# pps-lab/rofl-project-code

Hardware: AMD Instinct MI355X
Metric: range-proof elements/sec (create+verify), d=25k 32-bit (higher is better)
Workload: dtype u32x8 (255-bit integer field)

## Files before the change

### rofl_project_code_amd/csrc/host_msm.hpp

```cpp
#pragma once

MsmPlan msm_plan(size_t n, size_t np = 1) {
    MsmPlan p;
    static const size_t t13 = knob("ROFL_MSM_T13") ? (size_t)atol(knob("ROFL_MSM_T13")) : ((size_t)1 << 13);
    static const size_t t10_knob = knob("ROFL_MSM_T10") ? (size_t)atol(knob("ROFL_MSM_T10")) : 0;
    const size_t t10 = t10_knob ? t10_knob : (np >= 32 ? (size_t)1 << 11 : (size_t)1 << 9);
    if (n >= (1u << 17)) p.c = 16; else if (n >= t13) p.c = 13; else if (n >= t10) p.c = 10; else if (n >= 64) p.c = 7; else p.c = 4;
    if (const char *e = knob("ROFL_MSM_C")) { int v = atoi(e); if (v == 4 || v == 7 || v == 10 || v == 13 || v == 16) p.c = (u32)v; }
    p.W = (254 + p.c - 1) / p.c;
    p.W = (253 - p.c + p.c - 1) / p.c + 1;
    p.wide = (253 - p.c) - (p.c - 1) * (p.W - 1);
    p.B = 1u << (p.c - 1);
    p.levels = (p.c - 1) / 3;
    return p;
}
struct MsmOpt { u32 lr_nh = 0, lr_ng = 0; const niels *fb_wtab = nullptr; size_t fb_stride = 0; u32 fb_c = 16; std::function<void()> overlap; std::function<void(size_t)> post; u32 tag = 0;
                std::function<void(size_t, int)> post8;
                const sc *ip_dev = nullptr; u32 ip_nblk = 0; const niels *qpts = nullptr; bool *ip_included = nullptr;
                hipEvent_t pts_ready = nullptr; };

struct MsmAllow { bool fb = true, small = true, two = true, slots = true; };
enum class MsmKind { FixedBase, Small, Slots, CountSort };
struct MsmJob {
    MsmWs *ws = nullptr; size_t np = 0, nq = 0, n = 0, PW = 0; MsmPlan P{}; MsmKind kind = MsmKind::CountSort; bool lr = false, two = false, dev_horner = false;
// ... 8 lines not shown
    static const int sigmas = knob("ROFL_MSM_BIN_SIGMA") ? atoi(knob("ROFL_MSM_BIN_SIGMA")) : 8;
    size_t hot = 2 * avg, dev = 1;
    if (sigmas <= 0) return (u32)((hot + 256 + 63) / 64 * 64);
    while (dev * dev < hot) dev++;
    return (u32)((hot + (size_t)sigmas * dev + 64 + 63) / 64 * 64);
}

bool msm_plan_job(Ctx &C, MsmJob &J, const MsmOpt &opt, const MsmAllow &al, MsmMap &mm, u32 &small_cap, Msm2L &tl) {
    const size_t np = J.np, n = J.n; const bool lr = J.lr; const size_t nq = J.nq;
    const size_t per_side = lr ? n / 2 : n;
    mm = MsmMap{opt.lr_nh, opt.lr_ng, 0, 0, 0};
    J.two = false; J.sets = 0;
    bool want_fb = al.fb && opt.fb_wtab != nullptr && C.msm_slots;
    if (want_fb) {
        J.kind = MsmKind::FixedBase;
        J.P = msm_plan_c(opt.fb_c);
        bool crowded = C.crowded();
        size_t want = crowded ? C.msm_fb_threads / 2 : C.msm_fb_threads;
        u32 sets = J.P.W;
        for (u32 sdiv = 1; sdiv <= J.P.W; sdiv++)
            if (J.P.W % sdiv == 0 && (size_t)nq * (lr ? 2 : 1) * sdiv * J.P.B >= want) { sets = sdiv; break; }
        static const bool fitsets = !(knob("ROFL_MSM_FB_FITSETS") && atoi(knob("ROFL_MSM_FB_FITSETS")) == 0);
        if (fitsets && al.two && C.msm_two_level && (J.P.B == 32768 || J.P.B == 16384) && per_side >= 8192)
            while (sets < J.P.W && (size_t)msm_bin_cap(per_side * (J.P.W / sets) / 512) * 4 + 1024 > 96 * 1024) {
                u32 nx = sets + 1; while (nx < J.P.W && J.P.W % nx) nx++;
                sets = nx;
            }
        J.sets = sets;
        mm.fb_sets = sets; mm.fb_wps = J.P.W / sets; mm.fb_stride = (u32)opt.fb_stride;
        J.PW = nq * (lr ? 2 : 1) * sets;
        u32 cap = 16; while (cap < 2048 && (size_t)cap * J.P.B < 3 * per_side * (mm.fb_wps + 1)) cap *= 2;
        if (mm.fb_wps == 1) cap *= 2;
        J.cap = cap;
        bool two = al.two && C.msm_two_level && J.P.W * opt.fb_stride <= ((size_t)1 << 24) && (J.P.B == 32768 || J.P.B == 16384);
        const u32 fb0 = J.P.B == 32768 ? 7u : 6u;
        tl = Msm2L{256, fb0, 24, 0, 144};
        if (two) {
            auto size_bins = [&]() { tl.cap_bin = msm_bin_cap(per_side * mm.fb_wps / tl.nbins); return (size_t)tl.cap_bin * 4 + 1024 <= 96 * 1024; };
            bool fits = size_bins();
            if (!fits) { tl = Msm2L{512, fb0 - 1, 24, 0, 72}; fits = size_bins(); }
            if (!fits || per_side < 8192) two = false;
        }
        J.two = two;
        if (!two && (size_t)J.PW * J.P.B * J.cap * 4 > ((size_t)8 << 30)) return false;
        return true;
    }
    bool slots_mode = al.slots && C.msm_slots;
    J.P = msm_plan(n, J.np);
    if (C.msm_small_max && al.small && slots_mode && per_side <= C.msm_small_max && J.P.c > 10 && np * 26 <= 512) J.P = msm_plan_c(10);
    J.PW = np * J.P.W;
    { u32 cap = 16; while (cap < 256 && (size_t)cap * J.P.B < 4 * n) cap *= 2; J.cap = cap; }
    small_cap = per_side <= 8 * J.P.B ? (u32)MSM_SMALL_CAP : 72u;
    size_t small_lds = std::max((size_t)J.P.B * 4 * (1 + small_cap), std::max(((size_t)(J.P.B / 8) * 4 + (size_t)(J.P.B / 16) * 5 + 1) * sizeof(ge), ((size_t)J.P.B + (size_t)J.P.B * 3 / 4 + 1) * sizeof(ge)));
    bool small = slots_mode && al.small && C.msm_small_max && per_side <= C.msm_small_max && J.P.c <= 10 && per_side <= 16 * J.P.B && (J.PW <= 512 || small_lds <= 24 * 1024);
    J.kind = small ? MsmKind::Small : slots_mode ? MsmKind::Slots : MsmKind::CountSort;
    J.small_group = 1;
    if (small && J.P.B == 64 && J.PW > 512) {
        static const u32 grp = knob("ROFL_MSM_SMALL_GROUP") ? (u32)std::max(1, std::min(4, atoi(knob("ROFL_MSM_SMALL_GROUP")))) : 4u;
        J.small_group = grp == 3 ? 2 : grp;
    }
    if (J.kind == MsmKind::Slots && (size_t)J.PW * J.P.B * J.cap * 4 > ((size_t)8 << 30)) return false;
    return true;
}

MsmJob msm_enqueue(Ctx &C, MsmWs &W, const std::vector<MsmProb> &probs, size_t n, const MsmOpt &opt, MsmAllow &al, hipStream_t st = nullptr) {
    if (!st) st = C.stream;
    static const u32 acc_balance = knob("ROFL_ACC_BALANCE") ? (atoi(knob("ROFL_ACC_BALANCE")) ? 1u : 0u) : 1u;
    static const u32 dbg_mask = knob("ROFL_DBG_IDX_MASK") ? (u32)strtoul(knob("ROFL_DBG_IDX_MASK"), nullptr, 0) : 0x7fffffffu;
    static const u32 dbg_scatter = knob("ROFL_DBG_SCATTER") ? (u32)atoi(knob("ROFL_DBG_SCATTER")) : 0u;
    MsmJob J; J.ws = &W; J.np = probs.size(); J.n = n; J.lr = opt.lr_nh != 0; J.nq = J.lr ? J.np / 2 : J.np;
    const size_t np = J.np, nq = J.nq; const bool lr = J.lr;
    MsmMap mm{}; u32 small_cap = 0; Msm2L tl{};
    while (!msm_plan_job(C, J, opt, al, mm, small_cap, tl)) {
        if (al.fb && opt.fb_wtab && C.msm_slots) al.fb = false; else al.slots = false;
    }
    const MsmPlan &P = J.P; const size_t PW = J.PW; const bool fb = J.fb();
    MsmProb *d_probs = W.probs.as<MsmProb>(np);
    MsmProb *h_probs = W.h_probs.as<MsmProb>(np);
    for (size_t i = 0; i < np; i++) h_probs[i] = fb ? MsmProb{opt.fb_wtab, probs[i].scal} : probs[i];
    if (W.probs_on_dev.size() != np || memcmp(W.probs_on_dev.data(), h_probs, sizeof(MsmProb) * np) != 0) {
        HIPCHK(hipMemcpyAsync(d_probs, h_probs, sizeof(MsmProb) * np, hipMemcpyHostToDevice, st));
        W.probs_on_dev.assign(h_probs, h_probs + np);
    }
    u32 *cnt = W.cnt.as<u32>(PW * P.B + 4), *off = W.off.as<u32>(PW * P.B), *cur = W.cur.as<u32>(PW * P.B);
    u32 *perm = W.perm.as<u32>(PW * P.B);
    ge *buckets = W.buckets.as<ge>(PW * P.B);
    MsmWin mw{P.c, P.W, P.wide};
    static const bool host8_on = h8::available() && !(knob("ROFL_MSM_HOST8") && atoi(knob("ROFL_MSM_HOST8")) == 0);
    static const size_t host8_min = knob("ROFL_MSM_HOST8_MIN") ? (size_t)std::max(1L, atol(knob("ROFL_MSM_HOST8_MIN"))) : 8;
    J.dev_horner = !fb && P.W <= 64 && (np >= C.msm_dev_horner_min || (host8_on && np >= host8_min));
    J.host8 = J.dev_horner && host8_on;
    ge *hres_dev = W.h_res.dev<ge>(PW * (size_t)P.c + np);
    u32 *h_flag = W.h_ovf.as<u32>(4), *d_flag = W.h_ovf.dev<u32>(4);
    const u32 Wb = (u32)(PW / nq);
    const u32 n_side = (u32)(lr ? n / 2 : n);
    const u32 nb_final = P.c - 1;
    hipEvent_t e0 = nullptr, e1 = nullptr;
    *h_flag = 0;
    if (opt.ip_included) *opt.ip_included = J.kind == MsmKind::Small && opt.ip_dev && opt.qpts && lr;
    if (J.kind == MsmKind::Small) {
        ge *S_fin_s = J.dev_horner ? W.S[0].as<ge>(PW) : hres_dev;
        ge *C_fin_s = J.dev_horner ? W.Cacc[0].as<ge>(PW * (size_t)nb_final) : hres_dev + PW;
        const u32 G = J.small_group;
        size_t lds_lists = G > 1 ? (size_t)G * P.B * (4 + 2 * (size_t)small_cap)
                                 : (size_t)P.B * 4 * (1 + small_cap);
        size_t lds_red = G > 1 ? ((size_t)G * P.B * 3 / 4 + 1) * sizeof(ge)
                               : std::max(((size_t)(P.B / 8) * 4 + (size_t)(P.B / 16) * 5 + 1) * sizeof(ge), ((size_t)P.B + (size_t)P.B * 3 / 4 + 1) * sizeof(ge));
        uint64_t items = (uint64_t)np * n_side * P.W;
        KSpan ks(C.tm, st, ROFL_TK_MSM_SMALL, items * 7 + (uint64_t)PW * P.B * 10, (uint64_t)np * n_side * (32 + 96));
        static const bool small_tl = knob("ROFL_DBG_SMALL_TIMELINE") != nullptr;
        unsigned long long *tl_dev = nullptr;
        if (small_tl) { HIPCHK(hipMalloc(&tl_dev, PW * 32)); HIPCHK(hipMemsetAsync(tl_dev, 0, PW * 32, st)); }
        if (opt.pts_ready) HIPCHK(hipStreamWaitEvent(st, opt.pts_ready, 0));
        const u32 Wg = (P.W + G - 1) / G;
        if (G > 1)
            ROFL_LAUNCH(k_msm_small_g, dim3((unsigned)(np * Wg)), dim3(G * P.B), std::max(lds_lists, lds_red), st, n_side, mw, mm, d_probs, buckets,
                               S_fin_s, C_fin_s, nb_final, d_flag, small_cap, G, tl_dev, J.host8 ? hres_dev : (ge *)nullptr,
                               lr ? opt.ip_dev : (const sc *)nullptr, opt.ip_nblk, lr ? opt.qpts : (const niels *)nullptr);
        else
            ROFL_LAUNCH(k_msm_small, dim3((unsigned)PW), dim3(P.B < 64 ? 64 : P.B), std::max(lds_lists, lds_red), st, n_side, mw, mm, d_probs, buckets,
                               S_fin_s, C_fin_s, nb_final, d_flag, small_cap, G, tl_dev, J.host8 ? hres_dev : (ge *)nullptr,
                               lr ? opt.ip_dev : (const sc *)nullptr, opt.ip_nblk, lr ? opt.qpts : (const niels *)nullptr);
        if (small_tl) {
            std::vector<unsigned long long> hts(PW * 4);
            HIPCHK(hipMemcpyAsync(hts.data(), tl_dev, PW * 32, hipMemcpyDeviceToHost, st)); HIPCHK(hipStreamSynchronize(st)); HIPCHK(hipFree(tl_dev));
            double ph[3] = {0, 0, 0}; unsigned long long t_lo = ~0ull, t_hi = 0;
            const size_t nblocks = G > 1 ? np * Wg : PW;
            for (size_t b = 0; b < nblocks; b++) { for (int k = 0; k < 3; k++) ph[k] += (double)(hts[b * 4 + k + 1] - hts[b * 4 + k]); t_lo = std::min(t_lo, hts[b * 4]); t_hi = std::max(t_hi, hts[b * 4 + 3]); }
            fprintf(stderr, "[rofl] k_msm_small PW=%zu blocks=%zu n_side=%u c=%u: rank %.1f us, bucket sums %.1f us, reduce %.1f us (block means); first start -> last end %.1f us\n",
                    PW, nblocks, n_side, P.c, ph[0] / nblocks * 0.01, ph[1] / nblocks * 0.01, ph[2] / nblocks * 0.01, (double)(t_hi - t_lo) * 0.01);
        }
        if (J.host8) {}
        else if (J.dev_horner) ROFL_LAUNCH(k_msm_horner, dim3((unsigned)np), dim3(256), 0, st, mw, (const ge *)S_fin_s, (const ge *)C_fin_s, nb_final, hres_dev);
        return J;
    }
    const uint64_t terms = (uint64_t)(lr ? nq : np) * n;
    if (J.two) {
        u32 *bins = W.sorted.as<u32>(PW * tl.nbins * tl.cap_bin);
        u32 *bcur = W.cur.as<u32>(PW * tl.nbins * 2);
        u32 *btail = W.tail.as<u32>(PW * tl.nbins * (size_t)MSM_BIN_TAIL);
        HIPCHK(hipMemsetAsync(bcur, 0, sizeof(u32) * PW * tl.nbins * 2, st));
        static const bool worder_on = !(knob("ROFL_MSM_WINDOW_ORDER") && atoi(knob("ROFL_MSM_WINDOW_ORDER")) == 0);
        const u64 wdiv = (u64)mm.fb_stride * mm.fb_sets;
        const bool worder = worder_on && mm.fb_wps > 1 && mm.fb_wps <= 16 && wdiv && (wdiv & (wdiv - 1)) == 0 && wdiv < ((u64)1 << tl.ebits);
        const u32 worder_wps = worder ? mm.fb_wps : 1u, worder_shift = worder ? (u32)lg2u((size_t)wdiv) : 0u;
        u32 iter_pts = (tl.stage >= 144 ? 16384u : 12288u) / mm.fb_wps; if (iter_pts < 1024) iter_pts = 1024;
        u32 tile = iter_pts;
        while (((size_t)((n_side + tile - 1) / tile) * PW > 512 || (n_side + tile - 1) / tile > 48) && tile < n_side) tile *= 2;
        {
            static const bool tile_search = !(knob("ROFL_MSM_BIN_TILE_SEARCH") && atoi(knob("ROFL_MSM_BIN_TILE_SEARCH")) == 0);
            const size_t kCU = 256;
            auto cost = [&](u32 t) { const size_t tiles = (n_side + t - 1) / t; return (double)((tiles * PW + kCU - 1) / kCU) * ((double)std::min<u32>(t, n_side) + 0.25 * iter_pts); };
            if (tile_search) {
                u32 best = tile; double best_cost = cost(tile);
                for (u32 t = iter_pts; t < n_side + iter_pts; t += iter_pts) {
                    const size_t tiles = (n_side + t - 1) / t;
                    if (tiles > 48 || tiles * PW > 4096) continue;
                    const double c = cost(t);
                    if (c < best_cost * 0.999) { best = t; best_cost = c; }
                }
                if (knob("ROFL_TRACE")) fprintf(stderr, "[rofl] bin_l1 tiling: n_side=%u PW=%zu iter=%u: tile %u (%zu blocks, cost %.0f) -> best %u (%zu blocks, cost %.0f)\n", n_side, PW, iter_pts, tile,
                                                (size_t)((n_side + tile - 1) / tile) * PW, cost(tile), best, (size_t)((n_side + best - 1) / best) * PW, best_cost);
                if (best_cost < 0.85 * cost(tile)) tile = best;
            }
        }
        dim3 grid((n_side + tile - 1) / tile, (u32)PW);
        { KSpan ks(C.tm, st, ROFL_TK_MSM_SCATTER, 0, terms * 32 + terms * P.W * 4);
          ROFL_LAUNCH(k_msm_bin_l1, grid, dim3(1024), (size_t)(tl.nbins + tl.nbins * tl.stage) * 4, st, n_side, tile, iter_pts, mw, mm, d_probs, bcur, bins, btail, tl, d_flag);
          ROFL_LAUNCH(k_msm_bin_l2, dim3(tl.nbins, (u32)PW), dim3(512), (size_t)(2 * 128 * worder_wps + tl.cap_bin) * 4, st, tl, P.B, bcur, bins, (const u32 *)btail, cnt, off, d_flag,
                      worder_wps, worder_shift); }
        ROFL_LAUNCH(k_msm_scan, dim3((unsigned)PW), dim3(P.B >= 1024 ? 1024 : 256), 0, st, P.B, cnt, off, (u32 *)nullptr, perm);
        if (C.tm.enabled) { e0 = C.tm.get(); e1 = C.tm.get(); HIPCHK(hipEventRecord(e0, st)); }
        {
            HeavyScope heavy(C, st); hipStream_t hst = heavy.run;
            KSpan ks_acc(C.tm, hst, ROFL_TK_MSM_ACCUMULATE_FB, terms * P.W * 7, terms * 32);
            static const char *timeline = knob("ROFL_DBG_ACC_TIMELINE");
            if (timeline) {
                dim3 g = grid1((size_t)Wb * P.B, (u32)nq);
                size_t waves = (size_t)g.x * g.y * (TPB / 64);
                unsigned long long *rec; HIPCHK(hipMalloc(&rec, waves * 32)); HIPCHK(hipMemsetAsync(rec, 0, waves * 32, st));
                ROFL_LAUNCH(k_msm_accumulate_fb_dbg, g, dim3(TPB), 0, st, (u32)n, P.c, Wb, (u32)(np / nq), d_probs, cnt, off, bins, perm, buckets, MSM_LIST_ABS, dbg_mask, acc_balance, rec);
                std::vector<unsigned long long> h(waves * 4);
                HIPCHK(hipMemcpyAsync(h.data(), rec, waves * 32, hipMemcpyDeviceToHost, st)); HIPCHK(hipStreamSynchronize(st));
                if (FILE *f = fopen(timeline, "ab")) { unsigned long long hdr[4] = {0x54494d45ull, waves, g.x, g.y}; fwrite(hdr, 8, 4, f); fwrite(h.data(), 8, h.size(), f); fclose(f); }
                HIPCHK(hipFree(rec));
            } else
            ROFL_LAUNCH(k_msm_accumulate_fb, grid1((size_t)Wb * P.B, (u32)nq), dim3(TPB), 0, hst, (u32)n, P.c, Wb, (u32)(np / nq), d_probs, cnt, off, bins, perm, buckets, MSM_LIST_ABS, dbg_mask,
                        acc_balance | ((worder && nq > 1 && Wb > 1) ? 2u : 0u));
        }
        if (C.tm.enabled) HIPCHK(hipEventRecord(e1, st));
    } else if (J.kind != MsmKind::CountSort) {
        HIPCHK(hipMemsetAsync(cnt, 0, sizeof(u32) * (PW * P.B + 4), st));
        const u32 cap = J.cap;
        u32 *slots = W.sorted.as<u32>(PW * P.B * cap);
        MsmOvf *ovf = W.ovf.as<MsmOvf>(MSM_OVF_MAX);
        u32 *ovf_count = cnt + PW * P.B;
        if (C.msm_lds && n >= C.msm_lds_min && (size_t)P.B * 4 <= 128 * 1024) {
            u32 per_q = fb ? J.sets : P.W;
            u32 tile = n_side;
            u32 wps = fb ? mm.fb_wps : 1;
            while (tile > 1024 && ((size_t)tile * wps > (size_t)C.msm_lds_tile || (size_t)((n_side + tile - 1) / tile) * nq * (lr ? 2 : 1) * per_q < 256)) tile /= 2;
            dim3 grid((n_side + tile - 1) / tile, (u32)(nq * (lr ? 2 : 1) * per_q));
            uint64_t items = terms * P.W;
            KSpan ks(C.tm, st, ROFL_TK_MSM_SCATTER, 0, terms * 32 + items * 4);
            ROFL_LAUNCH(k_msm_scatter_lds, grid, dim3(1024), (size_t)P.B * 4, st, n_side, tile, mw, mm, d_probs, cnt, slots, cap, ovf_count, ovf, MSM_OVF_MAX, dbg_scatter);
        } else
            ROFL_LAUNCH(k_msm_scatter_slots, grid1(n, (u32)(nq * P.W)), dim3(TPB), 0, st, (u32)n, mw, mm, d_probs, cnt, slots, cap, ovf_count, ovf, MSM_OVF_MAX);
        ROFL_LAUNCH(k_msm_scan, dim3((unsigned)PW), dim3(P.B >= 1024 ? 1024 : 256), 0, st, P.B, cnt, off, (u32 *)nullptr, perm);
        if (opt.pts_ready) HIPCHK(hipStreamWaitEvent(st, opt.pts_ready, 0));
        if (C.tm.enabled) { e0 = C.tm.get(); e1 = C.tm.get(); HIPCHK(hipEventRecord(e0, st)); }
        {
            uint64_t acc_adds = terms * P.W;
            const bool big = acc_adds >= ((uint64_t)1 << 22);
            HeavyScope heavy(C, st, big); hipStream_t hst = heavy.run;
            KSpan ks_acc(C.tm, hst, fb ? ROFL_TK_MSM_ACCUMULATE_FB : ROFL_TK_MSM_ACCUMULATE_GEN, acc_adds * 7, terms * 32);
            if (fb) ROFL_LAUNCH(k_msm_accumulate_fb, grid1((size_t)Wb * P.B, (u32)nq), dim3(TPB), 0, hst, (u32)n, P.c, Wb, (u32)(np / nq), d_probs, cnt, off, slots, perm, buckets, cap, dbg_mask, acc_balance);
            else ROFL_LAUNCH(k_msm_accumulate_gen, grid1((size_t)Wb * P.B, (u32)nq), dim3(TPB), 0, hst, (u32)n, P.c, Wb, (u32)(np / nq), d_probs, cnt, off, slots, perm, buckets, cap, dbg_mask, acc_balance);
        }
        if (C.tm.enabled) HIPCHK(hipEventRecord(e1, st));
        ROFL_LAUNCH(k_msm_overflow, dim3(1), dim3(64), 0, st, Wb, P.B, (u32)(np / nq), d_probs, ovf_count, ovf, MSM_OVF_MAX, buckets, fb ? 1 : 0);
        HIPCHK(hipMemcpyAsync(h_flag, ovf_count, 4, hipMemcpyDeviceToHost, st));
    } else {
        HIPCHK(hipMemsetAsync(cnt, 0, sizeof(u32) * (PW * P.B + 4), st));
        u32 *sorted = W.sorted.as<u32>(PW * n * 2);
        ROFL_LAUNCH(k_msm_count, grid1(n, (u32)(nq * P.W)), dim3(TPB), 0, st, (u32)n, mw, mm, d_probs, cnt);
        ROFL_LAUNCH(k_msm_scan, dim3((unsigned)PW), dim3(P.B >= 1024 ? 1024 : 256), 0, st, P.B, cnt, off, cur, perm);
        ROFL_LAUNCH(k_msm_scatter, grid1(n, (u32)(nq * P.W)), dim3(TPB), 0, st, (u32)n, mw, mm, d_probs, cur, sorted);
        if (opt.pts_ready) HIPCHK(hipStreamWaitEvent(st, opt.pts_ready, 0));
        if (C.tm.enabled) { e0 = C.tm.get(); e1 = C.tm.get(); HIPCHK(hipEventRecord(e0, st)); }
        ROFL_LAUNCH(k_msm_accumulate_gen, grid1((size_t)Wb * P.B, (u32)nq), dim3(TPB), 0, st, (u32)n, P.c, Wb, (u32)(np / nq), d_probs, cnt, off, sorted, perm, buckets, 0u, dbg_mask, acc_balance);
        if (C.tm.enabled) HIPCHK(hipEventRecord(e1, st));
    }
    if (C.tm.enabled) {
        C.tm.acc_ev.push_back({e0, e1}); C.tm.t.msm_accumulate_launches++; C.tm.t.msm_additions += terms * P.W;
        char tg[96]; snprintf(tg, sizeof tg, "msm np=%zu n=%zu c=%u cap=%u fb=%u lr=%d", np, n, P.c, J.kind != MsmKind::CountSort ? J.cap : 0u, fb ? J.sets : 0u, (int)lr); C.tm.acc_tag.push_back(tg);
    }
    const ge *S_in = buckets; const ge *C_in = nullptr;
    u32 E = P.B, nb = 0, lv = 0;
    uint64_t red_adds = 0;
    { u32 e = P.B, b = 0; while (e > 512) { red_adds += (uint64_t)(e / 8) * (11 + 7 * b); e /= 8; b += 3; }
      red_adds += (uint64_t)(e / 8) * (16 + 7 * b); e /= 8; b += 3; while (e > 1) { red_adds += (uint64_t)(e / 2) * (1 + b); e /= 2; b++; } }
    ge *S_fin = J.dev_horner ? W.S[1].as<ge>(PW) : hres_dev;
    ge *C_fin = J.dev_horner ? W.Cacc[1].as<ge>(PW * (size_t)nb_final) : hres_dev + PW;
    {
        KSpan ks_red(C.tm, st, ROFL_TK_MSM_REDUCE, red_adds * PW * 9, (uint64_t)PW * P.B * 128);
        if (C.msm_group_reduce && P.B >= 1024) {
            u32 G = P.B / 512, gbits = P.c - 1 - 9;
            ge *GS = W.S[0].as<ge>(PW * G);
            ge *GC = W.Cacc[0].as<ge>(PW * (size_t)G * 9);
            size_t lds_a = ((size_t)64 * 4 + (size_t)32 * 5 + 1) * sizeof(ge);
            ROFL_LAUNCH(k_msm_reduce_fused, dim3((unsigned)(PW * G)), dim3(256), lds_a, st, 512u, 0u, (const ge *)buckets, (const ge *)nullptr, GS, GC, 9u);
            u32 half = G / 2 ? G / 2 : 1, nout = 10 + gbits;
            ROFL_LAUNCH(k_msm_reduce_groups, dim3((unsigned)PW), dim3(half, nout), (size_t)nout * half * sizeof(ge), st, G, gbits, (const ge *)GS, (const ge *)GC, S_fin, C_fin, nb_final);
        } else {
            while (E > 512) {
                u32 E8 = E / 8;
                ge *S_out = W.S[lv & 1].as<ge>(PW * E8);
                ge *C_out = W.Cacc[lv & 1].as<ge>(PW * (size_t)(nb + 3) * E8);
                static const int red_split = knob("ROFL_RED_SPLIT") ? atoi(knob("ROFL_RED_SPLIT")) : 0;
                ROFL_LAUNCH(k_msm_reduce_level, grid1((size_t)E8 * ((red_split ? 4 : 1) + nb), (u32)PW), dim3(TPB), 0, st, E, nb, S_in, C_in, S_out, C_out, red_split);
                S_in = S_out; C_in = C_out; E = E8; nb += 3; lv++;
            }
            if (J.dev_horner) { S_fin = W.S[lv & 1].as<ge>(PW); C_fin = W.Cacc[lv & 1].as<ge>(PW * (size_t)nb_final); }
            static const u32 red_fused_max = knob("ROFL_RED_FUSED_T") ? (u32)atoi(knob("ROFL_RED_FUSED_T")) : 768u;
            u32 fused_items = (E / 8) * (4 + nb), fused_threads = fused_items > 512 ? (fused_items > 640 ? 768 : 640) : fused_items > 256 ? 512 : fused_items > 128 ? 256 : fused_items > 64 ? 128 : 64;
            if (fused_threads > red_fused_max) fused_threads = red_fused_max;
            size_t lds = ((size_t)(E / 8) * (1 + nb + 3) + (size_t)(E / 16) * (1 + nb + 4) + 1) * sizeof(ge);
            ROFL_LAUNCH(k_msm_reduce_fused, dim3((unsigned)PW), dim3(fused_threads), lds, st, E, nb, S_in, C_in, S_fin, C_fin, nb_final);
        }
    }
    if (J.host8)
        ROFL_LAUNCH(k_msm_wsum, grid1(PW * 4), dim3(TPB), 0, st, (u32)PW, (const ge *)S_fin, (const ge *)C_fin, nb_final, hres_dev);
    else if (J.dev_horner)
        ROFL_LAUNCH(k_msm_horner, dim3((unsigned)np), dim3(256), 0, st, mw, (const ge *)S_fin, (const ge *)C_fin, nb_final, hres_dev);
    return J;
}

std::atomic<uint64_t> g_msm_stat[4];
bool msm_retry_inner(const MsmJob &J, MsmAllow &al);
bool msm_retry(const MsmJob &J, MsmAllow &al) {
    const bool small = J.kind == MsmKind::Small, two = J.two;
    const bool again = msm_retry_inner(J, al);
    g_msm_stat[again ? (small ? 1 : two ? 2 : 3) : 0].fetch_add(1, std::memory_order_relaxed);
    return again;
}
bool msm_retry_inner(const MsmJob &J, MsmAllow &al) {
    u32 flag = *J.ws->h_ovf.as<u32>(4);
    if (knob("ROFL_TRACE") && J.kind != MsmKind::CountSort) fprintf(stderr, "[rofl] msm np=%zu n=%zu c=%u cap=%u fb=%u lr=%d overflow=%u\n", J.np, J.n, J.P.c, J.cap, J.fb() ? J.sets : 0u, (int)J.lr, flag);
    if (J.kind == MsmKind::Small) { if (flag) { al.small = false; return true; } return false; }
    if (J.two) { if (flag) { al.two = false; return true; } return false; }
    if (J.kind == MsmKind::CountSort) return false;
    if (flag > MSM_OVF_MAX) { if (J.fb()) al.fb = false; else al.slots = false; return true; }
    return false;
}

void msm_finish(Ctx &C, const MsmJob &J, std::vector<ge5> &results, const MsmOpt &opt) {
    const size_t np = J.np, PW = J.PW; const MsmPlan &P = J.P; const u32 sets = J.sets;
    u32 nb = P.c - 1;
    ge *h = J.ws->h_res.as<ge>(PW * (size_t)P.c + np);
    double t0 = now_ms();
    results.resize(np);
    std::vector<double> cpu_each(np, 0.0);
    if (J.host8) {
        u32 pos[64];
        for (u32 w = 0; w < P.W; w++) pos[w] = w + 1 == P.W ? 253 - P.c : (w < P.wide ? w * P.c : P.wide * P.c + (w - P.wide) * (P.c - 1));
        C.pool->run((np + 7) / 8, [&](size_t b) {
            double tc0 = now_ms();
            size_t p0 = b * 8; int lanes = (int)std::min<size_t>(8, np - p0);
            ge5 out[8];
            h8::horner8(out, lanes, (int)P.W, pos, [&](int l, int w) { return (const ge *)&h[(p0 + (size_t)l) * P.W + (size_t)w]; });
            for (int l = 0; l < lanes; l++) results[p0 + l] = out[l];
            if (opt.post8) opt.post8(p0, lanes);
            else if (opt.post) for (int l = 0; l < lanes; l++) opt.post(p0 + l);
            cpu_each[p0] = now_ms() - tc0;
        });
    } else if (J.dev_horner) {
        if (opt.post) C.pool->run(np, [&](size_t p) { results[p] = h51::from_ge_loose(h[p]); opt.post(p); });
        else for (size_t p = 0; p < np; p++) results[p] = h51::from_ge_loose(h[p]);
    } else if (J.fb()) {
        auto fb_one = [&](size_t p) {
            size_t base = p * sets;
            ge5 acc = h51::identity(); bool started = false;
            for (int l = (int)nb - 1; l >= 0; l--) {
                if (started) acc = h51::gdouble(acc);
                for (u32 s = 0; s < sets; s++) { acc = h51::gadd(acc, h51::from_ge_loose(h[PW + (base + s) * nb + l])); started = true; }
                if (l == 0) for (u32 s = 0; s < sets; s++) acc = h51::gadd(acc, h51::from_ge_loose(h[base + s]));
            }
            results[p] = acc;
        };
// ... 107 lines not shown
```

### rofl_project_code_amd/csrc/host_rt.hpp

```cpp
#pragma once

struct Knob { const char *name, *dflt, *what; };
static const Knob KNOBS[] = {
    {"ROFL_LANES", "3", "calls that can be in flight on a device (HIP stream + workspace each); 1..16, larger values are clamped (with a note on stderr)"},
    {"ROFL_DEVICES", "0", "option devices: bit mask of the logical devices the batch entry points shard their clients over (0 = the calling thread's device only)"},
    {"ROFL_DEVICE_MAP", "", "logical -> physical HIP device, comma separated (0,0 = two logical devices on GPU 0: how the multi-device paths are tested on a one-GPU box); default: identity"},
    {"ROFL_RCCL_LIB", "librccl.so.1", "the RCCL library rofl_comm_* loads with dlopen (a host that has torch in the process names /opt/rocm/lib/librccl.so.1: the bare soname would resolve to torch's bundled copy)"},
    {"ROFL_HOST_THREADS", "usable cores, in [2, 16]", "threads of the primary lane's host pool (window combination, encodings, transcripts of a round); other lanes: usable cores, in [6, 12]"},
    {"ROFL_POOL_SPIN_US", "400", "how long an idle pool worker polls for the next job before it sleeps (0 = sleep at once)"},
    {"ROFL_BLOCKING_SYNC", "-1", "option blocking_sync: -1 spin while <= 3 calls are in flight, 0 always spin, 1 sleep between polls"},
    {"ROFL_VERIFY_ZIP_TRUNCATE", "0", "option verify_zip_truncate: 1 = the reference's zip-truncating verify_rangeproof"},
    {"ROFL_VERIFY_BATCH", "1", "option verify_batch: 0 = one check per proof, 1 = one per client, 2 = one per batch of clients (bisecting down to per-client checks on failure)"},
    {"ROFL_SIGMA_BATCH", "1", "option sigma_batch: 0 = one check per element in the Sigma-proof verifiers"},
    {"ROFL_STAGE_COHERENT", "0", "1 = the staging arenas are coherent (hipHostMallocDefault) pinned memory as in rounds 3-4 instead of non-coherent (the DMA engine reads 32 instead of 57 GB/s out of it)"},
    {"ROFL_STAGE_KEEP_MB", "256", "pinned staging memory a lane keeps between calls (a call that needed more frees it when it ends)"},
    {"ROFL_MSM_WINDOW_ORDER", "1", "0 = the bucket lists of the fixed-base two-level sort stay in arrival order and the accumulation's blocks in (problem, array) order (default: lists ordered by window slot, blocks array-major, so that the gathers of a launch stay within a few window slices of the table at a time)"},
    {"ROFL_SIGMA_SPLIT", "1", "0 = the per-element Sigma-proof prover runs as one thread per element (k_sigma_prove) instead of one thread per output point + a finishing kernel (k_sigma_points, k_sigma_finish); same bytes"},
    {"ROFL_MSM_BIN_TILE_SEARCH", "1", "0 = the coarse-bin pass of the two-level bucket sort keeps its power-of-two tile also when another tile length fills the CUs in fewer, shorter passes (batched rounds)"},
    {"ROFL_HEAVY_LO", "0", "1 = while several calls share the device, the chip-filling launches (bucket accumulation, generator folds) go to a lowest-priority stream of their lane so that other calls' short kernels are dispatched between their blocks (measured: neutral for rounds of range proofs, slower for rounds of L2 updates -- profiles/r06_experiments.txt item 2; off)"},
    {"ROFL_GENS_LAZY", "1", "0 = the first call of a shape waits for its full fold table (otherwise it is served from the compact table while a background thread builds the full one)"},
    {"ROFL_GENS_LAZY_IDLE_MS", "20", "the background build of a full fold table starts when no call has been in flight for this long (its allocation stalls every HIP call of the process)"},
    {"ROFL_GENS_LAZY_MAX_WAIT_MS", "3000", "... or after this long, whichever comes first (a host that never pauses still gets its full table)"},
    {"ROFL_GENS_RESERVE_MB", "40960", "HBM a table allocation of 4 GB or more leaves free on the device (other contexts / processes / workspaces; the runtime aborts when HBM runs out): the table is narrowed instead"},
    {"ROFL_GENS_BUDGET_MB", "131072", "HBM budget of the generator-table cache (LRU eviction of unpinned entries beyond it)"},
    {"ROFL_FOLD_T1", "3", "IPP rounds before the first generator fold (1..6)"},
    {"ROFL_FOLD_T", "2", "IPP rounds between later folds (1..6)"},
    {"ROFL_FOLD_MIN", "1024", "no fold once fewer generators per chunk would remain (launches with many chunks fold down to 64)"},
    {"ROFL_MSM_FB_FITSETS", "1", "0 = do not add bucket sets to a fixed-base launch whose coarse bins would not fit the two-level sort"},
    {"ROFL_MSM_BIN_SIGMA", "8", "room of a coarse bin of the two-level sort above twice its mean load, in standard deviations of that load (0 = the fixed 256 entries of rounds 2-3)"},
    {"ROFL_POOL_NAP", "1", "0 = pool workers do not nap through a wait whose length the caller announced (they poll for ROFL_POOL_SPIN_US, then sleep until woken)"},
    {"ROFL_SYNC_POLL", "0", "1 = wait for the lane's stream with hipStreamQuery in a pause loop instead of hipStreamSynchronize"},
    {"ROFL_FOLD_TAB", "1", "0 = first fold without the precomputed odd-multiple slices"},
    {"ROFL_FOLD_PB", "32", "piece width of the fold table in bits (16, 32, 64)"},
    {"ROFL_FOLD_W", "10", "NAF width of the fold table (3..10: 2^(w-2) odd multiples per 32-bit piece, 1/(w+1) of the digits non-zero; narrowed until the table fits ROFL_FOLD_TAB_MB)"},
    {"ROFL_FOLD_TAB_MB", "106496", "HBM budget of one (n, m) fold table (cfg 2 at width 10 and cfg 4 at width 9: 102.4 GB of the 288; 57344 = one width less, half the memory, +0.25 ms per cfg-2 proof)"},
    {"ROFL_FOLD_WNAF", "0", "later folds: NAF width over odd multiples of the sources built on a side stream during the preceding rounds (3..6; 0 = plain NAF over the sources alone: the build disturbs the rounds it runs beside by what the shorter fold chains save -- measured neutral, off by default)"},
    {"ROFL_FOLD_TAB_EV", "1", "0 = the first (table) fold scans digit arrays (k_fold_gens_tab) instead of walking an event list with operand prefetch (k_fold_gens_w)"},
    {"ROFL_FOLD_UNIT", "1", "0 = do not keep the common factor s_0 of a fold in gscale / hscale"},
    {"ROFL_FOLD_K", "0", "digit-position segments per fold output (1, 2, 4; 0 = by launch size)"},
    {"ROFL_FOLD_THREADS", "131072", "fold launches with fewer threads split their chains into segments"},
    {"ROFL_FOLD_DEFER", "1", "0 = the first fold converts every output to affine form itself (one inversion per output) instead of leaving that to k_niels_batch on the side stream"},
    {"ROFL_FOLD_REGS", "1", "0 = the generic fold kernel instead of the three-sources-in-registers one"},
    {"ROFL_IPP_FUSED", "1", "0 = k_ipp_fold_ab + k_ipp_scalars + k_ipp_inner instead of one k_ipp_round per round"},
    {"ROFL_MSM_LR", "1", "0 = separate L and R scalar arrays (with zeros) instead of the merged layout"},
    {"ROFL_MSM_FB", "1", "0 = no window tables (every MSM generic)"},
    {"ROFL_MSM_FB_MIN", "4096", "generator sets smaller than this get no window table"},
    {"ROFL_MSM_FB_C", "0", "one window width (13, 15, 16) for every window table; 0 = 16-bit tables, plus a 15-bit one for generator sets below 2^17 that launches with many problems and the verifier use"},
    {"ROFL_MSM_FB_THREADS", "524288", "accumulate threads a fixed-base launch aims for (decides the number of bucket sets)"},
    {"ROFL_MSM_TWO_LEVEL", "1", "0 = slot sort instead of the two-level bucket sort in fixed-base launches"},
    {"ROFL_MSM_SLOTS", "1", "0 = count / scan / scatter sort only (no fixed-capacity structures)"},
    {"ROFL_MSM_LDS", "1", "0 = per-item global atomics instead of LDS ranking in the slot sort"},
    {"ROFL_MSM_LDS_MIN", "8192", "MSMs with fewer terms use the per-item slot sort"},
    {"ROFL_MSM_LDS_TILE", "131072", "items one block of the LDS slot sort ranks"},
    {"ROFL_MSM_SMALL_MAX", "8192", "terms per side up to which a generic MSM runs as one fused launch (0 = off)"},
    {"ROFL_MSM_SMALL_GROUP", "4", "windows of a problem per block of the fused launch at c = 7 with more than 512 bucket arrays (1 = one window per one-wave block, 2, 4)"},
    {"ROFL_MERLIN_X8", "1", "0 = the verifier hashes every chunk's transcript prefix on its own even when the host has AVX-512 (eight chunks per instruction stream otherwise, from 32 chunks on)"},
    {"ROFL_MSM_HOST8", "1", "0 = launches with many problems combine their windows on the device (k_msm_horner) even when the host has AVX-512 IFMA"},
    {"ROFL_MSM_HOST8_MIN", "8", "launches with at least this many problems run their window chains eight per AVX-512 IFMA stream on the host (when the CPU has it)"},
    {"ROFL_MSM_FB_HOST8_MIN", "8", "fixed-base launches with at least this many problems finish eight problems per AVX-512 IFMA task (32 = as in rounds 3-4: one scalar chain per pool task below 32 problems)"},
    {"ROFL_KECCAK_ZMM", "", "host transcripts: 1 = Keccak-f[1600] with one state across five AVX-512 registers, 0 = the scalar rounds; unset = whichever a 50 us measurement at first use finds faster (Intel: the registers, 1.27x; Zen 5: scalar)"},
    {"ROFL_LR_FIRST", "1", "0 = l(x), r(x), the first round's MSM scalars and its inner products in three launches (k_lr_vec, k_ipp_scalars, k_ipp_inner) instead of one (k_lr_first)"},
    {"ROFL_HOP_CQ", "1", "0 = the <a,b> w B terms of a round are computed on the hop (after the wait) instead of on the pool while the round's MSM runs"},
    {"ROFL_MSM_DEV_HORNER_MIN", "32", "launches with at least this many problems combine their windows on the device"},
    {"ROFL_MSM_T13", "8192", "generic MSMs from this many terms on use 13-bit windows"},
    {"ROFL_MSM_T10", "512 / 2048", "generic MSMs from this many terms on use 10-bit windows (7-bit below, 4-bit below 64); default 2048 for launches with >= 32 problems"},
    {"ROFL_MSM_C", "0", "window width of every generic MSM (4, 7, 10, 13, 16; 0 = by size)"},
    {"ROFL_MSM_GROUP_REDUCE", "0", "1 = two-launch bucket reduction by groups of 512 (measured slower)"},
    {"ROFL_RED_SPLIT", "0", "1 = four threads per 8-group in k_msm_reduce_level (measured slower)"},
    {"ROFL_RED_FUSED_T", "768", "largest block of k_msm_reduce_fused"},
    {"ROFL_ACC_BALANCE", "1", "0 = accumulate blocks in plain descending-load order instead of equal-work blocks"},
    {"ROFL_TRACE", "0", "1 = one line per MSM on stderr, 2 = per-phase host timeline of every proof / verification"},
    {"ROFL_DBG_IDX_MASK", "0x7fffffff", "timing experiments only (WRONG results): confines the table gathers to a prefix"},
    {"ROFL_DBG_SCATTER", "0", "timing experiments only (WRONG results): 1 = no range reservation, 2 = no slot stores"},
    {"ROFL_DBG_SMALL_TIMELINE", "", "set: per-phase block timings of every fused small-MSM launch on stderr (synchronises; debugging)"},
    {"ROFL_DBG_ACC_TIMELINE", "", "file to append per-wave start / end / placement records of every fixed-base accumulate launch to"},
    {"ROFL_FEMUL_LDS", "0", "rofl_bench_femul: dynamic LDS per block (pins the micro-benchmark's occupancy)"},
    {"ROFL_FEMUL_MODE", "0", "rofl_bench_femul: 0 multiplication chain, 1-3 mixed addition from registers / a 32 KB table / a gathered table"},
    {"ROFL_FEMUL_TABLE", "2097152", "rofl_bench_femul mode 3: table entries (128 B each)"},
};
const char *knob(const char *name) {
#ifndef NDEBUG
    bool known = false; for (const Knob &k : KNOBS) known |= !strcmp(k.name, name);
    if (!known) { fprintf(stderr, "librofl_zk: unregistered knob %s\n", name); abort(); }
#endif
    return getenv(name);
}
static const bool g_keccak_knob_applied = [] { if (const char *e = knob("ROFL_KECCAK_ZMM")) if (*e) keccak_zmm_flag() = atoi(e) != 0 && __builtin_cpu_supports("avx512f"); return true; }();

thread_local std::string g_err;
int fail(int code, const std::string &msg) { g_err = msg; return code; }
struct HipErr { hipError_t e; const char *what; };
#define HIPCHK(x) do { hipError_t e__ = (x); if (e__ != hipSuccess) throw HipErr{e__, #x}; } while (0)
#define ROFL_LAUNCH(...) do { (void)hipGetLastError(); hipLaunchKernelGGL(__VA_ARGS__); hipError_t e__ = hipGetLastError(); \
                              if (e__ != hipSuccess && e__ != hipErrorNotReady) throw HipErr{e__, "kernel launch"}; } while (0)

double now_ms() { return std::chrono::duration<double, std::milli>(std::chrono::steady_clock::now().time_since_epoch()).count(); }

sc h_mont(const sc &canon) { return sc_to_mont(canon); }
sc h_canon(const sc &mont) { return sc_from_mont(mont); }
sc h_mul(const sc &a, const sc &b) { return sc_mul_plain(a, b); }
sc h_inv(const sc &canon) { return h_canon(h51::sc_invert_mont_fast(h_mont(canon))); }
bool sc_is_canonical_bytes(const uint8_t *b) { sc s = sc_frombytes(b); return !sc_geq_l(s.v); }

int sc_wnaf(int8_t out[256], const sc &k, unsigned w) {
    u32 x[9]; for (int i = 0; i < 8; i++) x[i] = k.v[i]; x[8] = 0;
    const int full = 1 << w, half = 1 << (w - 1);
    int top = -1;
    for (int pos = 0; pos < 256; pos++) {
        int d = 0;
        if (x[0] & 1) {
            d = (int)(x[0] & (u32)(full - 1)); if (d >= half) d -= full;
            if (d > 0) { x[0] -= (u32)d; }
            else { u64 c = (u64)(-d); for (int i = 0; i < 9 && c; i++) { c += x[i]; x[i] = (u32)c; c >>= 32; } }
            top = pos;
        }
        out[pos] = (int8_t)d;
        for (int i = 0; i < 8; i++) x[i] = (x[i] >> 1) | (x[i + 1] << 31);
        x[8] >>= 1;
    }
    return top;
}
int sc_naf(int8_t out[256], const sc &k) {
    u32 x[9]; for (int i = 0; i < 8; i++) x[i] = k.v[i]; x[8] = 0;
    int top = -1;
    for (int pos = 0; pos < 256; pos++) {
        int d = 0;
        if (x[0] & 1) {
            d = 2 - (int)(x[0] & 3);
            if (d > 0) { x[0] -= 1; }
            else { u64 c = 1; for (int i = 0; i < 9 && c; i++) { c += x[i]; x[i] = (u32)c; c >>= 32; } }
            top = pos;
        }
        out[pos] = (int8_t)d;
        for (int i = 0; i < 8; i++) x[i] = (x[i] >> 1) | (x[i + 1] << 31);
        x[8] >>= 1;
    }
    return top;
}

int wnaf_u64(int16_t out[FOLD_TAB_DIGITS], u64 piece, unsigned w) {
    unsigned __int128 k = piece; int top = -1;
    const int full = 1 << w, half = 1 << (w - 1);
    for (int pos = 0; pos < FOLD_TAB_DIGITS; pos++) {
        int d = 0;
        if (k & 1) { d = (int)(k & (unsigned)(full - 1)); if (d >= half) d -= full; if (d >= 0) k -= (unsigned)d; else k += (unsigned)(-d); top = pos; }
        out[pos] = (int16_t)d; k >>= 1;
    }
    return top;
}
// ... 815 lines not shown
```

### rofl_project_code_amd/csrc/kernels.hpp

```cpp
#pragma once
#include <type_traits>
#include "fe32.hpp"
#include "fe26.hpp"
#include "quad26.hpp"
#include "keccak.hpp"

namespace rofl {

#define TPB 256

#ifndef ROFL_KGROUP
#define ROFL_KGROUP 0
#endif
#define ROFL_KG(g) (ROFL_KGROUP == 0 || ROFL_KGROUP == (g))

typedef unsigned int v4u __attribute__((ext_vector_type(4)));
typedef __attribute__((address_space(1))) v4u g_uint4;
__device__ __forceinline__ niels gload_niels(const niels *p) {
    niels r;
    const g_uint4 *s = (const g_uint4 *)p;
    v4u *d = reinterpret_cast<v4u *>(&r);
#pragma unroll
    for (int i = 0; i < 6; i++) d[i] = s[i];
    return r;
// ... 1481 lines not shown
        E2 = E / 2;
        ge *so, *co;
        if (E2 == 1) { so = fin_s; co = fin_c; } else { so = bufs[sel]; co = bufs[sel] + E2; }
        msm_binary_level(E, nb, si, ci, so, co);
        __syncthreads();
        si = so; ci = co; E = E2; nb += 1; sel ^= 1;
    }
}
__device__ __forceinline__ void msm_binary_level_inplace(u32 E, u32 nb, ge *buf) {
    const u32 E2 = E / 2, items = E2 * (1 + nb);
    const ge *si = buf, *ci = buf + E;
    if (items * 4 <= blockDim.x) {
        const u32 item = threadIdx.x >> 2, q = threadIdx.x & 3;
        const bool on = item < items;
        const u32 role = on ? item / E2 : 0, g = on ? item % E2 : 0;
        fe res, hi;
        if (on) {
            const ge *pa, *pb;
            if (role == 0) { pa = &si[2 * g]; pb = &si[2 * g + 1]; }
            else { const ge *cc = ci + (size_t)(role - 1) * E; pa = &cc[2 * g]; pb = &cc[2 * g + 1]; }
            const fe fa = reinterpret_cast<const fe *>(pa)[q]; hi = reinterpret_cast<const fe *>(pb)[q];
            gq a, b; a.v = fd_unpack(fa); b.v = fd_unpack(hi);
            res = fd_pack(gq_add(a, b, q).v);
        }
        __syncthreads();
        if (on) {
            ge *so = buf, *co = buf + E2;
            ge *dst = role == 0 ? &so[g] : &co[(size_t)(role - 1) * E2 + g];
            reinterpret_cast<fe *>(dst)[q] = res;
            if (role == 0) reinterpret_cast<fe *>(&co[(size_t)nb * E2 + g])[q] = hi;
        }
        __syncthreads();
        return;
    }
    const u32 item = threadIdx.x;
    const bool on = item < items;
    const u32 role = on ? item / E2 : 0, g = on ? item % E2 : 0;
    ge res, hi;
    if (on) {
        const ge *cc = role == 0 ? si : ci + (size_t)(role - 1) * E;
        const ge lo = cc[2 * g]; hi = cc[2 * g + 1];
        res = gd_pack(gd_add(gd_unpack(lo), gd_unpack(hi)));
    }
    __syncthreads();
    if (on) {
        ge *so = buf, *co = buf + E2;
        if (role == 0) { so[g] = res; co[(size_t)nb * E2 + g] = hi; }
        else co[(size_t)(role - 1) * E2 + g] = res;
    }
    __syncthreads();
}
__device__ __forceinline__ void msm_reduce_binary_multi(u32 E, u32 G, u32 gv, const ge *si_g, ge *fin_s, ge *fin_c, u32 nb_final, unsigned char *smem) {
    ge *buf = reinterpret_cast<ge *>(smem);
    const u32 Et = G * E, E4 = Et / 4;
    {
        const u32 item = threadIdx.x;
        if (item < 3 * E4) {
            const u32 role = item / E4, g = item % E4;
            const u32 tree = (4 * g) / E, in_tree = (4 * g) % E, src_tree = tree < gv ? tree : gv - 1;
            const ge *b = si_g + (size_t)src_tree * E + in_tree;
            const ge x = load_ge(&b[role == 0 ? 0 : role == 1 ? 1 : 2]), y = load_ge(&b[role == 0 ? 1 : 3]);
            buf[(size_t)role * E4 + g] = gd_pack(gd_add(gd_unpack(x), gd_unpack(y)));
        }
        __syncthreads();
        if (4 * E4 <= blockDim.x) {
            const u32 g = threadIdx.x >> 2, q = threadIdx.x & 3;
            if (g < E4) {
                gq a, c; a.v = fd_unpack(reinterpret_cast<const fe *>(&buf[g])[q]); c.v = fd_unpack(reinterpret_cast<const fe *>(&buf[(size_t)2 * E4 + g])[q]);
                reinterpret_cast<fe *>(&buf[g])[q] = fd_pack(gq_add(a, c, q).v);
            }
        } else {
            for (u32 g = threadIdx.x; g < E4; g += blockDim.x) buf[g] = gd_pack(gd_add(gd_unpack(buf[g]), gd_unpack(buf[(size_t)2 * E4 + g])));
        }
        __syncthreads();
    }
    u32 nb = 2, Ecur = E4;
    while (Ecur > G) { msm_binary_level_inplace(Ecur, nb, buf); Ecur /= 2; nb += 1; }
    for (u32 item = threadIdx.x; item < gv * (1 + nb); item += blockDim.x) {
        const u32 g = item / (1 + nb), l = item % (1 + nb);
        if (l == 0) store_ge(&fin_s[g], buf[g]);
        else if (l - 1 < nb_final) store_ge(&fin_c[(size_t)g * nb_final + (l - 1)], buf[(size_t)G + (size_t)(l - 1) * G + g]);
    }
}
#define MSM_SMALL_CAP 64
#define MSM_SMALL_CAP_MAX 80
#if ROFL_KG(1)
template <bool L16>
__device__ __forceinline__ void msm_small_body(unsigned char *smem, u32 n_side, MsmWin mw, MsmMap mm, const MsmProb *probs, ge *buckets, ge *S_fin, ge *C_fin,
                                               u32 nb_final, u32 *overflow, u32 cap, u32 G, unsigned long long *dbg, ge *wsum_out,
                                               const sc *ip_dev, u32 ip_nblk, const niels *qpts) {
    auto stamp = [&](int k) { if (dbg && threadIdx.x == 0) dbg[(size_t)blockIdx.x * 4 + k] = wall_clock64(); };
    stamp(0);
    const u32 B = 1u << (mw.c - 1);
    const u32 Wg = (mw.W + G - 1) / G;
    const u32 p = G > 1 ? blockIdx.x / Wg : blockIdx.x / mw.W, w0 = G > 1 ? (blockIdx.x % Wg) * G : blockIdx.x % mw.W;
    const u32 gv = min(G, mw.W - w0);
    const u32 pw = p * mw.W + w0;
    const u32 VB = G * B;
    u32 side = mm.lr_nh ? (p & 1u) : 0u;
    typedef typename std::conditional<L16, unsigned short, u32>::type lst_t;
    const u32 SIGN = L16 ? 0x8000u : 0x80000000u, IDXM = SIGN - 1;
    u32 *lcnt = reinterpret_cast<u32 *>(smem);
    lst_t *lst = reinterpret_cast<lst_t *>(lcnt + VB);
    for (u32 b = threadIdx.x; b < VB; b += blockDim.x) lcnt[b] = 0;
    __syncthreads();
    const sc *scal = probs[p].scal;
    auto put = [&](const u32 *kw, u32 g, u32 entry_idx) {
        u32 wpos, wwid; msm_window(mw, w0 + g, wpos, wwid);
        int d = msm_digit_mem(kw, wpos, wwid);
        u32 ad = (u32)(d < 0 ? -d : d), entry = entry_idx | (d < 0 ? SIGN : 0u);
        for (int rep = 0; rep < 2; rep++) {
            u32 a1 = rep == 0 ? (ad > B ? B : 0u) : (ad > B ? ad - B : ad);
            if (!a1) continue;
            u32 vb = g * B + a1 - 1;
            u32 pos = atomicAdd(&lcnt[vb], 1u);
            if (pos < cap) lst[vb * cap + pos] = (lst_t)entry;
            else *(volatile u32 *)overflow = 1u;
        }
    };
    for (u32 k = threadIdx.x; k < n_side; k += blockDim.x) {
        u32 i = mm.lr_nh ? msm_side_term(mm, side, k) : k;
        const u32 *kw = reinterpret_cast<const u32 *>(&scal[i]);
        for (u32 g = 0; g < gv; g++) put(kw, g, i);
    }
    const u32 QIDX = IDXM;
    if (ip_dev && threadIdx.x == 0) {
        sc acc = sc_zero();
        for (u32 b = 0; b < ip_nblk; b++) acc = sc_add(acc, load_sc(&ip_dev[((size_t)(p >> 1) * ip_nblk + b) * 2 + (p & 1u)]));
        sc cs = sc_from_mont(acc);
        for (u32 g = 0; g < gv; g++) put(reinterpret_cast<const u32 *>(&cs), g, QIDX);
    }
    __syncthreads();
    stamp(1);
    const niels *pts = probs[p].pts;
    const niels *qpt = qpts ? qpts + (p >> 1) : pts;
    auto fetch = [&](u32 v) { const u32 i = v & IDXM; return gload_nd(i == QIDX ? qpt : &pts[i]); };
    u32 my_b = threadIdx.x;
    const bool sorted = (blockDim.x == 512 && B == 512) || G > 1;
    if (sorted) {
        __shared__ u32 chist[MSM_SMALL_CAP_MAX + 2], cbase[MSM_SMALL_CAP_MAX + 2];
        __shared__ unsigned short order[512];
        if (threadIdx.x < MSM_SMALL_CAP_MAX + 2) chist[threadIdx.x] = 0;
        __syncthreads();
        u32 mycnt = lcnt[threadIdx.x]; if (mycnt > cap) mycnt = cap;
        u32 rank_in = atomicAdd(&chist[mycnt], 1u);
        __syncthreads();
        if (threadIdx.x == 0) { u32 run = 0; for (int cval = (int)cap; cval >= 0; cval--) { cbase[cval] = run; run += chist[cval]; } }
        __syncthreads();
        order[cbase[mycnt] + rank_in] = (unsigned short)threadIdx.x;
        __syncthreads();
        u32 wv = threadIdx.x >> 6, ln = threadIdx.x & 63;
        u32 grp = G > 1 ? (wv + blockIdx.x) % G : (wv < 4 ? wv : 11 - wv);
        my_b = order[grp * 64 + ln];
    }
    for (u32 vb = my_b; vb < VB; vb += blockDim.x) {
        u32 num = lcnt[vb]; if (num > cap) num = cap;
        gd acc = gd_identity();
        u32 v = num ? lst[vb * cap] : 0u;
        nd nxt = fetch(v);
        for (u32 e = 0; e < num; e++) {
            nd q = nxt; bool ng = (v & SIGN) != 0;
            if (e + 1 < num) { v = lst[vb * cap + e + 1]; nxt = fetch(v); }
            acc = gd_madd(acc, q, ng);
        }
        if (vb < gv * B) store_gd(&buckets[(size_t)pw * B + vb], acc);
    }
// ... 768 lines not shown
```

Before: 1.164 million.

## Fuse fixed-base bucket reduction into one launch with last-block ticket combine

For fixed-base MSMs with 14/15-bit bucket counts, the three-launch bucket reduction chain is replaced by one kernel. Each block reduces a 1024-bucket slice to 11 partial outputs, and the last block per window, found through an atomic ticket, combines the slice partials into the window sum and binary-weighted terms. This is meant to cut launch overhead and intermediate global traffic. The cost is a grid of only PW*slices blocks and a serialized final combine done by one block.

```diff
diff --git a/rofl_project_code_amd/csrc/host_msm.hpp b/rofl_project_code_amd/csrc/host_msm.hpp
--- a/rofl_project_code_amd/csrc/host_msm.hpp
+++ b/rofl_project_code_amd/csrc/host_msm.hpp
@@ -114,7 +114,7 @@
         HIPCHK(hipMemcpyAsync(d_probs, h_probs, sizeof(MsmProb) * np, hipMemcpyHostToDevice, st));
         W.probs_on_dev.assign(h_probs, h_probs + np);
     }
-    u32 *cnt = W.cnt.as<u32>(PW * P.B + 4), *off = W.off.as<u32>(PW * P.B), *cur = W.cur.as<u32>(PW * P.B);
+    u32 *cnt = W.cnt.as<u32>(PW * P.B + 4 + PW), *off = W.off.as<u32>(PW * P.B), *cur = W.cur.as<u32>(PW * P.B);
     u32 *perm = W.perm.as<u32>(PW * P.B);
     ge *buckets = W.buckets.as<ge>(PW * P.B);
     MsmWin mw{P.c, P.W, P.wide};
@@ -127,6 +127,10 @@
     const u32 Wb = (u32)(PW / nq);
     const u32 n_side = (u32)(lr ? n / 2 : n);
     const u32 nb_final = P.c - 1;
+    static const bool red1_on = !(knob("ROFL_MSM_FB_REDUCE1") && atoi(knob("ROFL_MSM_FB_REDUCE1")) == 0);
+    const bool red1 = red1_on && fb && !J.dev_horner && (P.B == 32768 || P.B == 16384) && nb_final == 10 + lg2u(P.B / MSM_RED1_T) &&
+                      PW * (P.B / MSM_RED1_T) <= 512;
+    u32 *tickets = nullptr;
     hipEvent_t e0 = nullptr, e1 = nullptr;
     *h_flag = 0;
     if (opt.ip_included) *opt.ip_included = J.kind == MsmKind::Small && opt.ip_dev && opt.qpts && lr;
@@ -169,9 +173,11 @@
     const uint64_t terms = (uint64_t)(lr ? nq : np) * n;
     if (J.two) {
         u32 *bins = W.sorted.as<u32>(PW * tl.nbins * tl.cap_bin);
-        u32 *bcur = W.cur.as<u32>(PW * tl.nbins * 2);
+        const size_t nbc = PW * tl.nbins * 2 + (red1 ? PW : 0);
+        u32 *bcur = W.cur.as<u32>(nbc);
         u32 *btail = W.tail.as<u32>(PW * tl.nbins * (size_t)MSM_BIN_TAIL);
-        HIPCHK(hipMemsetAsync(bcur, 0, sizeof(u32) * PW * tl.nbins * 2, st));
+        HIPCHK(hipMemsetAsync(bcur, 0, sizeof(u32) * nbc, st));
+        if (red1) tickets = bcur + PW * tl.nbins * 2;
         static const bool worder_on = !(knob("ROFL_MSM_WINDOW_ORDER") && atoi(knob("ROFL_MSM_WINDOW_ORDER")) == 0);
         const u64 wdiv = (u64)mm.fb_stride * mm.fb_sets;
         const bool worder = worder_on && mm.fb_wps > 1 && mm.fb_wps <= 16 && wdiv && (wdiv & (wdiv - 1)) == 0 && wdiv < ((u64)1 << tl.ebits);
@@ -222,7 +228,8 @@
         }
         if (C.tm.enabled) HIPCHK(hipEventRecord(e1, st));
     } else if (J.kind != MsmKind::CountSort) {
-        HIPCHK(hipMemsetAsync(cnt, 0, sizeof(u32) * (PW * P.B + 4), st));
+        HIPCHK(hipMemsetAsync(cnt, 0, sizeof(u32) * (PW * P.B + 4 + (red1 ? PW : 0)), st));
+        if (red1) tickets = cnt + PW * P.B + 4;
         const u32 cap = J.cap;
         u32 *slots = W.sorted.as<u32>(PW * P.B * cap);
         MsmOvf *ovf = W.ovf.as<MsmOvf>(MSM_OVF_MAX);
@@ -276,7 +283,11 @@
     ge *C_fin = J.dev_horner ? W.Cacc[1].as<ge>(PW * (size_t)nb_final) : hres_dev + PW;
     {
         KSpan ks_red(C.tm, st, ROFL_TK_MSM_REDUCE, red_adds * PW * 9, (uint64_t)PW * P.B * 128);
-        if (C.msm_group_reduce && P.B >= 1024) {
+        if (red1) {
+            ge *part = W.S[0].as<ge>(PW * (size_t)(P.B / MSM_RED1_T) * 11);
+            ROFL_LAUNCH(k_msm_reduce_fb1, dim3(P.B / MSM_RED1_T, (u32)PW), dim3(256), (size_t)512 * sizeof(ge), st, P.B, (const ge *)buckets, part, tickets,
+                        S_fin, C_fin, nb_final);
+        } else if (C.msm_group_reduce && P.B >= 1024) {
             u32 G = P.B / 512, gbits = P.c - 1 - 9;
             ge *GS = W.S[0].as<ge>(PW * G);
             ge *GC = W.Cacc[0].as<ge>(PW * (size_t)G * 9);
diff --git a/rofl_project_code_amd/csrc/host_rt.hpp b/rofl_project_code_amd/csrc/host_rt.hpp
--- a/rofl_project_code_amd/csrc/host_rt.hpp
+++ b/rofl_project_code_amd/csrc/host_rt.hpp
@@ -65,6 +65,7 @@
     {"ROFL_MSM_T13", "8192", "generic MSMs from this many terms on use 13-bit windows"},
     {"ROFL_MSM_T10", "512 / 2048", "generic MSMs from this many terms on use 10-bit windows (7-bit below, 4-bit below 64); default 2048 for launches with >= 32 problems"},
     {"ROFL_MSM_C", "0", "window width of every generic MSM (4, 7, 10, 13, 16; 0 = by size)"},
+    {"ROFL_MSM_FB_REDUCE1", "1", "0 = fixed-base bucket reduction as the chain of three launches (k_msm_reduce_level x 2, k_msm_reduce_fused) instead of one (k_msm_reduce_fb1)"},
     {"ROFL_MSM_GROUP_REDUCE", "0", "1 = two-launch bucket reduction by groups of 512 (measured slower)"},
     {"ROFL_RED_SPLIT", "0", "1 = four threads per 8-group in k_msm_reduce_level (measured slower)"},
     {"ROFL_RED_FUSED_T", "768", "largest block of k_msm_reduce_fused"},
diff --git a/rofl_project_code_amd/csrc/kernels.hpp b/rofl_project_code_amd/csrc/kernels.hpp
--- a/rofl_project_code_amd/csrc/kernels.hpp
+++ b/rofl_project_code_amd/csrc/kernels.hpp
@@ -1587,6 +1587,75 @@
         else if (l - 1 < nb_final) store_ge(&fin_c[(size_t)g * nb_final + (l - 1)], buf[(size_t)G + (size_t)(l - 1) * G + g]);
     }
 }
+#define MSM_RED1_T 1024u
+#if ROFL_KG(1)
+__global__ void __launch_bounds__(256, 2) k_msm_reduce_fb1(u32 E, const ge *buckets, ge *part , u32 *tickets ,
+                                                          ge *S_fin, ge *C_fin, u32 nb_final) {
+    extern __shared__ __align__(16) unsigned char smem[];
+    ge *buf = reinterpret_cast<ge *>(smem);
+    __shared__ u32 is_last;
+    const u32 pw = blockIdx.y, g = blockIdx.x, nsl = gridDim.x, t = threadIdx.x;
+    const ge *sl_b = buckets + (size_t)pw * E + (size_t)g * MSM_RED1_T;
+    for (u32 item = t; item < 512; item += 256) {
+        const u32 role = item >> 7, gg = item & 127;
+        const ge *s = sl_b + (size_t)gg * 8;
+        const u32 i0 = role == 0 ? 0u : role == 1 ? 1u : role == 2 ? 2u : 4u;
+        const u32 i1 = role == 0 ? 1u : role == 3 ? 5u : 3u;
+        const u32 i2 = role == 0 ? 2u : role == 1 ? 5u : 6u;
+        const u32 i3 = role == 0 ? 3u : 7u;
+        gd acc = gd_add(load_gd(&s[i0]), load_gd(&s[i1]));
+        acc = gd_add(acc, load_gd(&s[i2]));
+        acc = gd_add(acc, load_gd(&s[i3]));
+        buf[item] = gd_pack(acc);
+    }
+    __syncthreads();
+    for (u32 gg = t >> 2; gg < 128; gg += 64) {
+        const u32 q = t & 3;
+        gq a, c; a.v = fd_unpack(reinterpret_cast<const fe *>(&buf[gg])[q]); c.v = fd_unpack(reinterpret_cast<const fe *>(&buf[384 + gg])[q]);
+        reinterpret_cast<fe *>(&buf[gg])[q] = fd_pack(gq_add(a, c, q).v);
+    }
+    __syncthreads();
+    u32 Ecur = 128, nb = 3;
+    while (Ecur > 1) { msm_binary_level_inplace(Ecur, nb, buf); Ecur /= 2; nb += 1; }
+    ge *my = part + ((size_t)pw * nsl + g) * 11;
+    if (t < 11) store_ge(&my[t], buf[t]);
+    __threadfence();
+    __syncthreads();
+    if (t == 0) {
+        const u32 k = atomicAdd(&tickets[pw], 1u);
+        is_last = k == nsl - 1;
+        if (is_last) atomicExch(&tickets[pw], 0u);
+    }
+    __syncthreads();
+    if (!is_last) return;
+    __threadfence();
+    const u32 nout = 11 + (31 - __clz(nsl));
+    const ge *pp = part + (size_t)pw * nsl * 11;
+    {
+        const u32 o = t >> 4, j = t & 15;
+        gd acc = gd_identity();
+        if (o < nout)
+            for (u32 sl = j; sl < nsl; sl += 16) {
+                if (o < 11) acc = gd_add(acc, load_gd(&pp[(size_t)sl * 11 + o]));
+                else if ((sl >> (o - 11)) & 1u) acc = gd_add(acc, load_gd(&pp[(size_t)sl * 11]));
+            }
+        buf[t] = gd_pack(acc);
+    }
+    __syncthreads();
+    for (u32 h = 8; h >= 1; h >>= 1) {
+        for (u32 it = t >> 2; it < nout * h; it += 64) {
+            const u32 o = it / h, j = it % h, q = t & 3;
+            gq a, c; a.v = fd_unpack(reinterpret_cast<const fe *>(&buf[o * 16 + j])[q]); c.v = fd_unpack(reinterpret_cast<const fe *>(&buf[o * 16 + j + h])[q]);
+            reinterpret_cast<fe *>(&buf[o * 16 + j])[q] = fd_pack(gq_add(a, c, q).v);
+        }
+        __syncthreads();
+    }
+    if (t < nout) {
+        if (t == 0) store_ge(&S_fin[pw], buf[0]);
+        else if (t - 1 < nb_final) store_ge(&C_fin[(size_t)pw * nb_final + (t - 1)], buf[t * 16]);
+    }
+}
+#endif
 #define MSM_SMALL_CAP 64
 #define MSM_SMALL_CAP_MAX 80
 #if ROFL_KG(1)
```

Measured after the change: 1.179 million (median of 5 runs). 1.3% higher.
